# zubair-irshad/HunyuanWorld-Mirror

Hardware: AMD Instinct MI355X
Metric: views/sec (higher is better)
Workload: dtype bf16; 1 GPU; 8-view 518x518 bf16, no priors, camera+depth+pointmap+normal heads, 8 views/GPU, full 1.23B-param arch; views_per_gpu=8, global_views=8, parallelism=view-shard x1, collective=none (1 GPU)

## Files before the change

hunyuanworld-mirror_amd/csrc/elementwise.hip:

```cpp
#include "wm_common.h"
#include "wm_kernels.h"

namespace {

constexpr float RESNET_MEAN[3] = {0.485f, 0.456f, 0.406f};
constexpr float RESNET_STD[3] = {0.229f, 0.224f, 0.225f};

template <int NV>
__global__ __launch_bounds__(256) void layernorm_kernel(const WmLnArgs p) {
  const int lane = threadIdx.x & 63;
  const long long row = (long long)blockIdx.x * 4 + (threadIdx.x >> 6);
  const long long nrows = (long long)p.groups * p.rows_per_group;
  if (row >= nrows) return;
  const int g = (int)(row / p.rows_per_group), q = (int)(row - (long long)g * p.rows_per_group);
  const float* x = p.x + ((size_t)g * p.in_group + p.in_off + q) * p.ld_in;
  const size_t orow = (size_t)g * p.out_group + p.out_off + q;
  float4 v[NV];
  float s = 0.f;
#pragma unroll
  for (int i = 0; i < NV; ++i) {
    const int c = (i * 64 + lane) * 4;
    v[i] = c < p.D ? *(const float4*)(x + c) : make_float4(0, 0, 0, 0);
    s += v[i].x + v[i].y + v[i].z + v[i].w;
  }
// ... 153 lines not shown
#pragma unroll
        for (int i = 0; i < 4; ++i) {
          const float o = __shfl_xor(v[i], 4);
          v[i] = v[i] * c[i] + sign * o * s[i];
        }
      }
      if (which == 0) {
#pragma unroll
        for (int i = 0; i < 4; ++i) v[i] *= p.q_scale;
      }
    }
    uint2 u;
    u.x = (uint32_t)f2t<T>(v[0]) | ((uint32_t)f2t<T>(v[1]) << 16);
    u.y = (uint32_t)f2t<T>(v[2]) | ((uint32_t)f2t<T>(v[3]) << 16);
    u16* dst = (u16*)(which == 0 ? p.q : which == 1 ? p.k : p.v);
    if (head_ok) *(uint2*)(dst + obase) = u;
  }
}

template <int T>
__global__ __launch_bounds__(256) void im2col_kernel(const float* __restrict__ img, u16* __restrict__ out, int N, int C,
                                                     int H, int W, int ps, int Kpad, int normalize) {
  const int gh = H / ps, gw = W / ps, K = C * ps * ps;
  const size_t total = (size_t)N * gh * gw * Kpad;
  for (size_t i = (size_t)blockIdx.x * 256 + threadIdx.x; i < total; i += (size_t)gridDim.x * 256) {
    const int k = (int)(i % Kpad);
    const size_t r = i / Kpad;
    float v = 0.f;
    if (k < K) {
      const int c = k / (ps * ps), kk = k - c * ps * ps, ky = kk / ps, kx = kk - ky * ps;
      const int px = (int)(r % gw), py = (int)((r / gw) % gh), n = (int)(r / ((size_t)gw * gh));
      v = img[(((size_t)n * C + c) * H + py * ps + ky) * W + px * ps + kx];
      if (normalize) v = (v - RESNET_MEAN[c]) / RESNET_STD[c];
    }
    out[i] = f2t<T>(v);
  }
}

template <int T>
WM_NO_PACKED_FP32 __global__ __launch_bounds__(256) void im2col_rows_kernel(const float* __restrict__ img, u16* __restrict__ out, int N, int C,
                                                          int H, int W, int ps, int Kpad, int normalize) {
  extern __shared__ __attribute__((aligned(16))) u16 tile[];
  const int gh = H / ps, gw = W / ps, K = C * ps * ps;
  const int c = blockIdx.x % C, py = (blockIdx.x / C) % gh, n = blockIdx.x / (C * gh);
  const float mean = normalize ? RESNET_MEAN[c] : 0.f, sd = normalize ? RESNET_STD[c] : 1.f;
  const float* src = img + (((size_t)n * C + c) * H + (size_t)py * ps) * W;
  const int half = (ps * W) >> 1;
  for (int i = threadIdx.x; i < half; i += 256) {
    const float2 v = *(const float2*)(src + 2 * i);
    const float a = normalize ? (v.x - mean) / sd : v.x, b = normalize ? (v.y - mean) / sd : v.y;
    *(uint32_t*)(tile + 2 * i) = (uint32_t)f2t<T>(a) | ((uint32_t)f2t<T>(b) << 16);
  }
  __syncthreads();
  const int pp = ps * ps, hp = pp >> 1;
  u16* dst = out + ((size_t)n * gh * gw + (size_t)py * gw) * Kpad + (size_t)c * pp;
  for (int i = threadIdx.x; i < gw * hp; i += 256) {
    const int px = i / hp, kk = 2 * (i - px * hp), ky = kk / ps, kx = kk - ky * ps;
    *(uint32_t*)(dst + (size_t)px * Kpad + kk) = *(const uint32_t*)(tile + ky * W + px * ps + kx);
  }
  if (c == C - 1) {
    const int tail = (Kpad - K) >> 1;
    u16* z = out + ((size_t)n * gh * gw + (size_t)py * gw) * Kpad + K;
    for (int i = threadIdx.x; i < gw * tail; i += 256) {
      const int px = i / tail, j = i - px * tail;
      *(uint32_t*)(z + (size_t)px * Kpad + 2 * j) = 0u;
    }
  }
}

template <int T>
__global__ __launch_bounds__(256) void im2col7_kernel(const float* __restrict__ img, u16* __restrict__ out, int N, int H, int W,
                                                      int Kpad) {
  const size_t total = (size_t)N * H * W * Kpad;
  for (size_t i = (size_t)blockIdx.x * 256 + threadIdx.x; i < total; i += (size_t)gridDim.x * 256) {
    const int k = (int)(i % Kpad);
    const size_t r = i / Kpad;
    float v = 0.f;
    if (k < 147) {
      const int c = k / 49, kk = k - c * 49, ky = kk / 7, kx = kk - ky * 7;
      const int x = (int)(r % W), y = (int)((r / W) % H), n = (int)(r / ((size_t)W * H));
      const int iy = y + ky - 3, ix = x + kx - 3;
      if (iy >= 0 && iy < H && ix >= 0 && ix < W) v = img[(((size_t)n * 3 + c) * H + iy) * W + ix];
    }
    out[i] = f2t<T>(v);
  }
}

__global__ __launch_bounds__(256) void gs_splat_kernel(const float* __restrict__ gp, const float* __restrict__ img,
                                                       const float* __restrict__ depth, const float* __restrict__ cam,
                                                       float* __restrict__ means, float* __restrict__ quats,
                                                       float* __restrict__ scales, float* __restrict__ opac,
                                                       float* __restrict__ sh, float* __restrict__ wts, int N, int H, int W, int dbg) {
  const size_t npix = (size_t)N * H * W;
  for (size_t i = (size_t)blockIdx.x * 256 + threadIdx.x; i < npix; i += (size_t)gridDim.x * 256) {
    const int x = (int)(i % W), y = (int)((i / W) % H), n = (int)(i / ((size_t)W * H));
    const float* g = gp + i * 12;
    const float4 g0 = *(const float4*)g, g1 = *(const float4*)(g + 4), g2 = *(const float4*)(g + 8);
    const float qn = sqrtf(g0.x * g0.x + g0.y * g0.y + g0.z * g0.z + g0.w * g0.w) + 1e-8f;
    quats[i * 4 + 0] = g0.x / qn; quats[i * 4 + 1] = g0.y / qn; quats[i * 4 + 2] = g0.z / qn; quats[i * 4 + 3] = g0.w / qn;
    const float e0 = expf(g1.x), e1 = expf(g1.y), e2 = expf(g1.z);
    scales[i * 3 + 0] = e0 > 0.3f ? 0.3f : e0; scales[i * 3 + 1] = e1 > 0.3f ? 0.3f : e1; scales[i * 3 + 2] = e2 > 0.3f ? 0.3f : e2;
    opac[i] = 1.0f / (1.0f + expf(-g1.w));
    const float C0 = 0.28209479177387814f;
    const size_t hw = (size_t)H * W, p0 = (size_t)n * 3 * hw + (size_t)y * W + x;
    sh[i * 3 + 0] = (img[p0] - 0.5f) / C0 + g2.x;
    sh[i * 3 + 1] = (img[p0 + hw] - 0.5f) / C0 + g2.y;
    sh[i * 3 + 2] = (img[p0 + 2 * hw] - 0.5f) / C0 + g2.z;
    wts[i] = 1.0f / (1.0f + expf(-g2.w));
    const float* v = cam + n * 9;
    const float qi = v[3], qj = v[4], qk = v[5], qr = v[6];
    const float s2 = 2.0f / (qi * qi + qj * qj + qk * qk + qr * qr);
    const float R[9] = {1 - s2 * (qj * qj + qk * qk), s2 * (qi * qj - qk * qr), s2 * (qi * qk + qj * qr),
                        s2 * (qi * qj + qk * qr), 1 - s2 * (qi * qi + qk * qk), s2 * (qj * qk - qi * qr),
                        s2 * (qi * qk - qj * qr), s2 * (qj * qk + qi * qr), 1 - s2 * (qi * qi + qj * qj)};
    const float fy = H * 0.5f / tanf(v[7] * 0.5f), fx = W * 0.5f / tanf(v[8] * 0.5f);
    const float d = depth[i];
    const float xc = ((float)x - W * 0.5f) * d / fx, yc = ((float)y - H * 0.5f) * d / fy, zc = d;
    float tc[3];
    for (int a = 0; a < 3; ++a) tc[a] = -(R[0 * 3 + a] * v[0] + R[1 * 3 + a] * v[1] + R[2 * 3 + a] * v[2]);
    for (int a = 0; a < 3; ++a) means[i * 3 + a] = R[0 * 3 + a] * xc + R[1 * 3 + a] * yc + R[2 * 3 + a] * zc + tc[a];
#ifdef WM_DBG_SPLAT_BUILD
    if (dbg) {
      opac[i] = v[0]; wts[i] = v[1]; scales[i * 3 + 0] = v[2]; scales[i * 3 + 1] = v[7]; scales[i * 3 + 2] = v[8];
      quats[i * 4 + 0] = v[3]; quats[i * 4 + 1] = v[4]; quats[i * 4 + 2] = v[5]; quats[i * 4 + 3] = v[6];
      sh[i * 3 + 0] = tc[0]; sh[i * 3 + 1] = tc[1]; sh[i * 3 + 2] = tc[2];
    }
#else
    (void)dbg;
#endif
  }
}

__global__ __launch_bounds__(256) void dino_special_kernel(const float* cls, const float* reg, const float* pos, float* X,
                                                           int N, int T, int R, int D) {
  const int total = N * (1 + R) * D;
  for (int i = blockIdx.x * 256 + threadIdx.x; i < total; i += gridDim.x * 256) {
    const int d = i % D, t = (i / D) % (1 + R), n = i / (D * (1 + R));
    X[((size_t)n * T + t) * D + d] = t == 0 ? cls[d] + pos[d] : reg[(t - 1) * D + d];
  }
}

__global__ __launch_bounds__(256) void vgt_special_kernel(float* X, const float* cam, const float* reg, const float* pose,
                                                          const float* ray, int N, int P, int R, int D, int cond,
                                                          int first_view_global) {
  const int psi = 1 + R + (cond ? 2 : 0);
  const int total = N * psi * D;
  for (int i = blockIdx.x * 256 + threadIdx.x; i < total; i += gridDim.x * 256) {
    const int d = i % D, t = (i / D) % psi, n = i / (D * psi);
    const int slot = (first_view_global + n) == 0 ? 0 : 1;
    float v;
    if (t == 0) v = cam[slot * D + d];
    else if (t <= R) v = reg[(slot * R + (t - 1)) * D + d];
    else if (t == R + 1) v = pose ? pose[(size_t)n * D + d] : 0.f;
    else v = ray ? ray[(size_t)n * D + d] : 0.f;
    X[((size_t)n * P + t) * D + d] = v;
  }
}

__global__ __launch_bounds__(256) void copy2d_kernel(const float* __restrict__ src, float* __restrict__ dst, int rows,
                                                     int cols4, int ld_src, int ld_dst) {
  const size_t total = (size_t)rows * cols4;
  for (size_t i = (size_t)blockIdx.x * 256 + threadIdx.x; i < total; i += (size_t)gridDim.x * 256) {
    const size_t r = i / cols4;
    const int c = (int)(i - r * cols4) * 4;
    *(float4*)(dst + r * ld_dst + c) = *(const float4*)(src + r * ld_src + c);
  }
}

template <int OUT16>
__global__ __launch_bounds__(256) void bilinear_kernel(const float* __restrict__ in, void* __restrict__ outp, int N, int Hi,
                                                       int Wi, int Ho, int Wo, int C4, const float* __restrict__ addx,
                                                       const float* __restrict__ addy) {
  const float sy = Ho > 1 ? (float)(Hi - 1) / (float)(Ho - 1) : 0.f;
  const float sx = Wo > 1 ? (float)(Wi - 1) / (float)(Wo - 1) : 0.f;
  const size_t total = (size_t)N * Ho * Wo * C4;
  for (size_t i = (size_t)blockIdx.x * 256 + threadIdx.x; i < total; i += (size_t)gridDim.x * 256) {
    const int c = (int)(i % C4) * 4;
    size_t r = i / C4;
    const int x = (int)(r % Wo); r /= Wo;
    const int y = (int)(r % Ho);
    const int n = (int)(r / Ho);
    const float fy = sy * y, fx = sx * x;
    int y0 = (int)fy, x0 = (int)fx;
    y0 = y0 < Hi - 1 ? y0 : Hi - 1;
    x0 = x0 < Wi - 1 ? x0 : Wi - 1;
    const int y1 = y0 < Hi - 1 ? y0 + 1 : y0, x1 = x0 < Wi - 1 ? x0 + 1 : x0;
    const float wy = fy - y0, wx = fx - x0;
    const size_t C = (size_t)C4 * 4;
    const float* b = in + (size_t)n * Hi * Wi * C + c;
    const float4 v00 = *(const float4*)(b + ((size_t)y0 * Wi + x0) * C);
    const float4 v01 = *(const float4*)(b + ((size_t)y0 * Wi + x1) * C);
    const float4 v10 = *(const float4*)(b + ((size_t)y1 * Wi + x0) * C);
    const float4 v11 = *(const float4*)(b + ((size_t)y1 * Wi + x1) * C);
    const float w00 = (1.f - wy) * (1.f - wx), w01 = (1.f - wy) * wx, w10 = wy * (1.f - wx), w11 = wy * wx;
    float4 o;
    o.x = w00 * v00.x + w01 * v01.x + w10 * v10.x + w11 * v11.x;
    o.y = w00 * v00.y + w01 * v01.y + w10 * v10.y + w11 * v11.y;
    o.z = w00 * v00.z + w01 * v01.z + w10 * v10.z + w11 * v11.z;
    o.w = w00 * v00.w + w01 * v01.w + w10 * v10.w + w11 * v11.w;
    if (addx) {
      const int half = (int)(C >> 1);
      const float4 a = c < half ? *(const float4*)(addx + (size_t)x * half + c) : *(const float4*)(addy + (size_t)y * half + (c - half));
      o.x += a.x; o.y += a.y; o.z += a.z; o.w += a.w;
    }
    const size_t oi = (((size_t)n * Ho + y) * Wo + x) * C + c;
    if constexpr (OUT16 == 0) {
      *(float4*)((float*)outp + oi) = o;
    } else {
      uint2 u;
      if constexpr (OUT16 == 1) { u.x = (uint32_t)f2bf(o.x) | ((uint32_t)f2bf(o.y) << 16); u.y = (uint32_t)f2bf(o.z) | ((uint32_t)f2bf(o.w) << 16); }
      else { u.x = (uint32_t)f2h(o.x) | ((uint32_t)f2h(o.y) << 16); u.y = (uint32_t)f2h(o.z) | ((uint32_t)f2h(o.w) << 16); }
      *(uint2*)((u16*)outp + oi) = u;
    }
  }
}

constexpr int RT_P = 12;
template <int OUT16>
__global__ __launch_bounds__(256) void bilinear_tiled_kernel(const float* __restrict__ in, void* __restrict__ outp, int N, int Hi, int Wi,
                                                             int Ho, int Wo, int C, const float* __restrict__ addx,
                                                             const float* __restrict__ addy) {
  __shared__ __attribute__((aligned(16))) float patch[RT_P * RT_P * 64];
  const float sy = Ho > 1 ? (float)(Hi - 1) / (float)(Ho - 1) : 0.f;
  const float sx = Wo > 1 ? (float)(Wi - 1) / (float)(Wo - 1) : 0.f;
  const int tiles_x = (Wo + 15) / 16, tiles_y = (Ho + 15) / 16;
  int t = blockIdx.x;
  const int tx = t % tiles_x; t /= tiles_x;
  const int ty = t % tiles_y;
  const int n = t / tiles_y;
  const int y0 = ty * 16, x0 = tx * 16;
  const int y_last = min(y0 + 15, Ho - 1), x_last = min(x0 + 15, Wo - 1);
  auto lo = [](float s, int o, int lim) { int v = (int)(s * o); return v < lim - 1 ? v : lim - 1; };
  const int py0 = lo(sy, y0, Hi), px0 = lo(sx, x0, Wi);
  const int py1 = min(lo(sy, y_last, Hi) + 1, Hi - 1), px1 = min(lo(sx, x_last, Wi) + 1, Wi - 1);
  const int ph = py1 - py0 + 1, pw = px1 - px0 + 1;
  const int tid = threadIdx.x;
  const float* src = in + (size_t)n * Hi * Wi * C;
  for (int c0 = 0; c0 < C; c0 += 64) {
    __syncthreads();
    const int npieces = ph * pw * 16;
    for (int q = tid; q < npieces; q += 256) {
      const int pix = q >> 4, k = q & 15;
      const int yy = pix / pw, xx = pix - yy * pw;
      *(float4*)(patch + pix * 64 + k * 4) = *(const float4*)(src + ((size_t)(py0 + yy) * Wi + (px0 + xx)) * C + c0 + k * 4);
    }
    __syncthreads();
#pragma unroll 2
    for (int it = 0; it < 8; ++it) {
      const int item = it * 256 + tid, pix = item >> 3, g = item & 7;
      const int y = y0 + (pix >> 4), x = x0 + (pix & 15);
      if (y >= Ho || x >= Wo) continue;
      const float fy = sy * y, fx = sx * x;
      int ya = (int)fy, xa = (int)fx;
      ya = ya < Hi - 1 ? ya : Hi - 1;
      xa = xa < Wi - 1 ? xa : Wi - 1;
      const int yb = ya < Hi - 1 ? ya + 1 : ya, xb = xa < Wi - 1 ? xa + 1 : xa;
      const float wy = fy - ya, wx = fx - xa;
      const float w00 = (1.f - wy) * (1.f - wx), w01 = (1.f - wy) * wx, w10 = wy * (1.f - wx), w11 = wy * wx;
      const float* p00 = patch + ((ya - py0) * pw + (xa - px0)) * 64 + g * 8;
      const float* p01 = patch + ((ya - py0) * pw + (xb - px0)) * 64 + g * 8;
      const float* p10 = patch + ((yb - py0) * pw + (xa - px0)) * 64 + g * 8;
      const float* p11 = patch + ((yb - py0) * pw + (xb - px0)) * 64 + g * 8;
      float o[8];
#pragma unroll
      for (int h = 0; h < 2; ++h) {
        const float4 v00 = *(const float4*)(p00 + 4 * h), v01 = *(const float4*)(p01 + 4 * h);
        const float4 v10 = *(const float4*)(p10 + 4 * h), v11 = *(const float4*)(p11 + 4 * h);
        o[4 * h + 0] = w00 * v00.x + w01 * v01.x + w10 * v10.x + w11 * v11.x;
        o[4 * h + 1] = w00 * v00.y + w01 * v01.y + w10 * v10.y + w11 * v11.y;
        o[4 * h + 2] = w00 * v00.z + w01 * v01.z + w10 * v10.z + w11 * v11.z;
        o[4 * h + 3] = w00 * v00.w + w01 * v01.w + w10 * v10.w + w11 * v11.w;
      }
      const int c = c0 + g * 8;
      if (addx) {
        const int half = C >> 1;
        const float* a = c < half ? addx + (size_t)x * half + c : addy + (size_t)y * half + (c - half);
        const float4 a0 = *(const float4*)a, a1 = *(const float4*)(a + 4);
        o[0] += a0.x; o[1] += a0.y; o[2] += a0.z; o[3] += a0.w; o[4] += a1.x; o[5] += a1.y; o[6] += a1.z; o[7] += a1.w;
      }
      const size_t oi = (((size_t)n * Ho + y) * Wo + x) * C + c;
      if constexpr (OUT16 == 0) {
        *(float4*)((float*)outp + oi) = make_float4(o[0], o[1], o[2], o[3]);
        *(float4*)((float*)outp + oi + 4) = make_float4(o[4], o[5], o[6], o[7]);
      } else {
        uint4 u;
        if constexpr (OUT16 == 1) {
          u.x = (uint32_t)f2bf(o[0]) | ((uint32_t)f2bf(o[1]) << 16); u.y = (uint32_t)f2bf(o[2]) | ((uint32_t)f2bf(o[3]) << 16);
          u.z = (uint32_t)f2bf(o[4]) | ((uint32_t)f2bf(o[5]) << 16); u.w = (uint32_t)f2bf(o[6]) | ((uint32_t)f2bf(o[7]) << 16);
        } else {
          u.x = (uint32_t)f2h(o[0]) | ((uint32_t)f2h(o[1]) << 16); u.y = (uint32_t)f2h(o[2]) | ((uint32_t)f2h(o[3]) << 16);
          u.z = (uint32_t)f2h(o[4]) | ((uint32_t)f2h(o[5]) << 16); u.w = (uint32_t)f2h(o[6]) | ((uint32_t)f2h(o[7]) << 16);
        }
        *(uint4*)((u16*)outp + oi) = u;
      }
    }
  }
}
static bool bilinear_tiled_ok(int Hi, int Wi, int Ho, int Wo, int C) {
  if (C % 64 || Ho < 16 || Wo < 16) return false;
  const float sy = Ho > 1 ? (float)(Hi - 1) / (float)(Ho - 1) : 0.f, sx = Wo > 1 ? (float)(Wi - 1) / (float)(Wo - 1) : 0.f;
  return 15.f * sy + 3.f <= (float)RT_P && 15.f * sx + 3.f <= (float)RT_P;
}

__global__ __launch_bounds__(256) void add_kernel(const float* __restrict__ a, const float* __restrict__ b,
                                                  float* __restrict__ o, size_t n4) {
  for (size_t i = (size_t)blockIdx.x * 256 + threadIdx.x; i < n4; i += (size_t)gridDim.x * 256) {
    const float4 x = ((const float4*)a)[i], y = ((const float4*)b)[i];
    ((float4*)o)[i] = make_float4(x.x + y.x, x.y + y.y, x.z + y.z, x.w + y.w);
  }
}

__global__ __launch_bounds__(256) void dpt_tail_kernel(const float* __restrict__ y32, const float* __restrict__ w,
                                                       const float* __restrict__ b, float* __restrict__ attr,
                                                       float* __restrict__ conf, size_t npix, int C, int act) {
  __shared__ float sw[4 * 32 + 4];
  if (threadIdx.x < C * 32) sw[threadIdx.x] = w[threadIdx.x];
  if (threadIdx.x < C) sw[128 + threadIdx.x] = b[threadIdx.x];
  __syncthreads();
  for (size_t i = (size_t)blockIdx.x * 256 + threadIdx.x; i < npix; i += (size_t)gridDim.x * 256) {
    float o[4] = {sw[128], sw[129], sw[130], sw[131]};
    const float4* src = (const float4*)(y32 + i * 32);
#pragma unroll
    for (int k = 0; k < 8; ++k) {
      float4 v = src[k];
      v.x = relu_keep_nan(v.x); v.y = relu_keep_nan(v.y); v.z = relu_keep_nan(v.z); v.w = relu_keep_nan(v.w);
#pragma unroll
      for (int c = 0; c < 4; ++c)
        if (c < C) o[c] += v.x * sw[c * 32 + 4 * k] + v.y * sw[c * 32 + 4 * k + 1] + v.z * sw[c * 32 + 4 * k + 2] + v.w * sw[c * 32 + 4 * k + 3];
    }
    const int A = C - 1;
    if (act == WM_ACT_NORM) {
      float nn = 0.f;
      for (int c = 0; c < A; ++c) nn += o[c] * o[c];
      nn = sqrtf(nn);
      for (int c = 0; c < A; ++c) attr[i * A + c] = o[c] / nn;
    } else if (act == WM_ACT_EXP) {
      for (int c = 0; c < A; ++c) attr[i * A + c] = expf(o[c]);
    } else {
      for (int c = 0; c < A; ++c) attr[i * A + c] = inv_log(o[c]);
    }
    conf[i] = 1.0f + expf(o[A]);
  }
}

inline int grid_for(size_t n, int per_block = 256) {
  size_t g = (n + per_block - 1) / per_block;
  return (int)(g < 1 ? 1 : (g > 2048 ? 2048 : g));
}

}

hipError_t wm_launch_layernorm(const WmLnArgs& a, hipStream_t s) {
  const long long rows = (long long)a.groups * a.rows_per_group;
  if (rows <= 0) return hipSuccess;
  if (a.D % 4 || a.D > 2048 || a.ld_in % 4 || a.ld_out % 4) return hipErrorInvalidValue;
  dim3 grid((unsigned)((rows + 3) / 4)), block(256);
  const int nv = (a.D + 255) / 256;
  if (a.D == nv * 256 && (nv == 4 || nv == 8) && !a.w && !a.b && !a.out_f32) {
    if (nv == 4) {
      if (a.dtype == WM_T_BF16) hipLaunchKernelGGL((layernorm_fast_noaffine_kernel<4, WM_T_BF16>), grid, block, 0, s, a);
      else hipLaunchKernelGGL((layernorm_fast_noaffine_kernel<4, WM_T_F16>), grid, block, 0, s, a);
    } else {
      if (a.dtype == WM_T_BF16) hipLaunchKernelGGL((layernorm_fast_noaffine_kernel<8, WM_T_BF16>), grid, block, 0, s, a);
      else hipLaunchKernelGGL((layernorm_fast_noaffine_kernel<8, WM_T_F16>), grid, block, 0, s, a);
    }
    return hipGetLastError();
  }
  if (a.D == nv * 256 && (nv == 4 || nv == 8) && a.w && a.b && !a.out_f32) {
    const int rpw = nv == 4 && wm_tune(WM_TUNE_LN_RPW, 1) == 2 ? 2 : 1;
    const dim3 g2((unsigned)((rows + 4 * rpw - 1) / (4 * rpw)));
    if (nv == 4 && rpw == 2) {
      if (a.dtype == WM_T_BF16) hipLaunchKernelGGL((layernorm_fast_kernel<4, WM_T_BF16, 2>), g2, block, 0, s, a);
      else hipLaunchKernelGGL((layernorm_fast_kernel<4, WM_T_F16, 2>), g2, block, 0, s, a);
    } else if (nv == 4) {
      if (a.dtype == WM_T_BF16) hipLaunchKernelGGL((layernorm_fast_kernel<4, WM_T_BF16, 1>), grid, block, 0, s, a);
      else hipLaunchKernelGGL((layernorm_fast_kernel<4, WM_T_F16, 1>), grid, block, 0, s, a);
    } else {
      if (a.dtype == WM_T_BF16) hipLaunchKernelGGL((layernorm_fast_kernel<8, WM_T_BF16, 1>), grid, block, 0, s, a);
      else hipLaunchKernelGGL((layernorm_fast_kernel<8, WM_T_F16, 1>), grid, block, 0, s, a);
    }
    return hipGetLastError();
  }
  if (nv <= 1) hipLaunchKernelGGL(layernorm_kernel<1>, grid, block, 0, s, a);
  else if (nv <= 2) hipLaunchKernelGGL(layernorm_kernel<2>, grid, block, 0, s, a);
  else if (nv <= 4) hipLaunchKernelGGL(layernorm_kernel<4>, grid, block, 0, s, a);
  else hipLaunchKernelGGL(layernorm_kernel<8>, grid, block, 0, s, a);
  return hipGetLastError();
}

hipError_t wm_launch_qkv_post(const WmQkvArgs& a, hipStream_t s) {
  if (a.M <= 0) return hipSuccess;
  const long long waves = (long long)a.M * ((a.H + 3) / 4);
  dim3 grid((unsigned)((waves + 3) / 4)), block(256);
  if (a.dtype == WM_T_BF16) hipLaunchKernelGGL(qkv_post_kernel<WM_T_BF16>, grid, block, 0, s, a);
  else hipLaunchKernelGGL(qkv_post_kernel<WM_T_F16>, grid, block, 0, s, a);
  return hipGetLastError();
}

hipError_t wm_launch_im2col(const float* img, void* out, int N, int C, int H, int W, int ps, int Kpad, int normalize,
                            int dtype, hipStream_t s) {
  const size_t total = (size_t)N * (H / ps) * (W / ps) * Kpad;
  if (!total) return hipSuccess;
  const size_t lds = (size_t)ps * W * sizeof(u16);
  if (ps % 2 == 0 && W % 2 == 0 && (C * ps * ps) % 2 == 0 && Kpad % 2 == 0 && lds <= 64 * 1024) {
    const dim3 grid((unsigned)(N * (H / ps) * C));
    if (dtype == WM_T_BF16) hipLaunchKernelGGL(im2col_rows_kernel<WM_T_BF16>, grid, dim3(256), lds, s, img, (u16*)out, N, C, H, W, ps, Kpad, normalize);
    else hipLaunchKernelGGL(im2col_rows_kernel<WM_T_F16>, grid, dim3(256), lds, s, img, (u16*)out, N, C, H, W, ps, Kpad, normalize);
    return hipGetLastError();
  }
  if (dtype == WM_T_BF16)
    hipLaunchKernelGGL(im2col_kernel<WM_T_BF16>, dim3(grid_for(total)), dim3(256), 0, s, img, (u16*)out, N, C, H, W, ps, Kpad, normalize);
  else
    hipLaunchKernelGGL(im2col_kernel<WM_T_F16>, dim3(grid_for(total)), dim3(256), 0, s, img, (u16*)out, N, C, H, W, ps, Kpad, normalize);
  return hipGetLastError();
}

hipError_t wm_launch_im2col7(const float* img, void* out, int N, int H, int W, int Kpad, int dtype, hipStream_t s) {
  const size_t total = (size_t)N * H * W * Kpad;
  if (!total) return hipSuccess;
  if (dtype == WM_T_BF16) hipLaunchKernelGGL(im2col7_kernel<WM_T_BF16>, dim3(grid_for(total)), dim3(256), 0, s, img, (u16*)out, N, H, W, Kpad);
  else hipLaunchKernelGGL(im2col7_kernel<WM_T_F16>, dim3(grid_for(total)), dim3(256), 0, s, img, (u16*)out, N, H, W, Kpad);
  return hipGetLastError();
}

hipError_t wm_launch_gs_splat(const float* gp, const float* img, const float* depth, const float* cam, float* means, float* quats,
                              float* scales, float* opac, float* sh, float* wts, int N, int H, int W, hipStream_t s) {
  if (!N) return hipSuccess;
#ifdef WM_DBG_SPLAT_BUILD
  const int dbg = wm_tune(WM_TUNE_DBG_SPLAT, 0) ? 1 : 0;
#else
  const int dbg = 0;
#endif
  hipLaunchKernelGGL(gs_splat_kernel, dim3(grid_for((size_t)N * H * W)), dim3(256), 0, s, gp, img, depth, cam, means, quats, scales,
                     opac, sh, wts, N, H, W, dbg);
  return hipGetLastError();
}

hipError_t wm_launch_dino_tokens(const float* , const float* cls, const float* reg, const float* pos, float* X,
                                 int N, int hw, int R, int D, hipStream_t s) {
  hipLaunchKernelGGL(dino_special_kernel, dim3(grid_for((size_t)N * (1 + R) * D)), dim3(256), 0, s, cls, reg, pos, X, N,
                     1 + R + hw, R, D);
  return hipGetLastError();
}

hipError_t wm_launch_vgt_special(float* X, const float* cam_tok, const float* reg_tok, const float* pose_tok,
                                 const float* ray_tok, int N, int P, int R, int D, int cond, int first_view_global,
                                 hipStream_t s) {
  hipLaunchKernelGGL(vgt_special_kernel, dim3(grid_for((size_t)N * (3 + R) * D)), dim3(256), 0, s, X, cam_tok, reg_tok,
                     pose_tok, ray_tok, N, P, R, D, cond, first_view_global);
  return hipGetLastError();
}

hipError_t wm_launch_copy2d(const float* src, float* dst, int rows, int cols, int ld_src, int ld_dst, hipStream_t s) {
  if (cols % 4 || ld_src % 4 || ld_dst % 4) return hipErrorInvalidValue;
  if (!rows) return hipSuccess;
  hipLaunchKernelGGL(copy2d_kernel, dim3(grid_for((size_t)rows * cols / 4)), dim3(256), 0, s, src, dst, rows, cols / 4, ld_src, ld_dst);
  return hipGetLastError();
}

hipError_t wm_launch_bilinear(const float* in, float* out, int N, int Hi, int Wi, int Ho, int Wo, int C, const float* addx,
                              const float* addy, hipStream_t s) {
  if (C % 8) return hipErrorInvalidValue;
  const size_t total = (size_t)N * Ho * Wo * (C / 4);
  if (!total) return hipSuccess;
  if (bilinear_tiled_ok(Hi, Wi, Ho, Wo, C)) {
    hipLaunchKernelGGL(bilinear_tiled_kernel<0>, dim3((unsigned)(N * ((Ho + 15) / 16) * ((Wo + 15) / 16))), dim3(256), 0, s, in, (void*)out, N, Hi, Wi, Ho, Wo, C, addx, addy);
    return hipGetLastError();
  }
  hipLaunchKernelGGL(bilinear_kernel<0>, dim3(grid_for(total)), dim3(256), 0, s, in, (void*)out, N, Hi, Wi, Ho, Wo, C / 4, addx, addy);
  return hipGetLastError();
}

hipError_t wm_launch_bilinear16(const float* in, void* out16, int N, int Hi, int Wi, int Ho, int Wo, int C, const float* addx,
                                const float* addy, int dtype, hipStream_t s) {
  if (C % 4) return hipErrorInvalidValue;
  const size_t total = (size_t)N * Ho * Wo * (C / 4);
  if (!total) return hipSuccess;
  if (bilinear_tiled_ok(Hi, Wi, Ho, Wo, C)) {
    const dim3 grid((unsigned)(N * ((Ho + 15) / 16) * ((Wo + 15) / 16)));
    if (dtype == WM_T_BF16) hipLaunchKernelGGL(bilinear_tiled_kernel<1>, grid, dim3(256), 0, s, in, out16, N, Hi, Wi, Ho, Wo, C, addx, addy);
    else hipLaunchKernelGGL(bilinear_tiled_kernel<2>, grid, dim3(256), 0, s, in, out16, N, Hi, Wi, Ho, Wo, C, addx, addy);
    return hipGetLastError();
  }
  if (dtype == WM_T_BF16) hipLaunchKernelGGL(bilinear_kernel<1>, dim3(grid_for(total)), dim3(256), 0, s, in, out16, N, Hi, Wi, Ho, Wo, C / 4, addx, addy);
  else hipLaunchKernelGGL(bilinear_kernel<2>, dim3(grid_for(total)), dim3(256), 0, s, in, out16, N, Hi, Wi, Ho, Wo, C / 4, addx, addy);
  return hipGetLastError();
}

hipError_t wm_launch_add(const float* a, const float* b, float* out, size_t n, hipStream_t s) {
  if (n % 4) return hipErrorInvalidValue;
  if (!n) return hipSuccess;
  hipLaunchKernelGGL(add_kernel, dim3(grid_for(n / 4)), dim3(256), 0, s, a, b, out, n / 4);
  return hipGetLastError();
}

template <int VEC>
__global__ __launch_bounds__(256) void depth_to_world_kernel(const float* __restrict__ depth, const float* __restrict__ ext,
                                                             const float* __restrict__ intr, float* __restrict__ world,
                                                             float* __restrict__ cam, unsigned char* __restrict__ mask, int B,
                                                             int H, int W, float eps) {
  const size_t hw = (size_t)H * W, total = (size_t)B * hw / VEC;
  for (size_t i = (size_t)blockIdx.x * 256 + threadIdx.x; i < total; i += (size_t)gridDim.x * 256) {
    float zz[VEC], cw[3 * VEC], cc[3 * VEC];
    if constexpr (VEC == 4) {
      const float4 d4 = *(const float4*)(depth + 4 * i);
      zz[0] = d4.x; zz[1] = d4.y; zz[2] = d4.z; zz[3] = d4.w;
    } else {
      zz[0] = depth[i];
    }
    unsigned int mbits = 0;
#pragma unroll
    for (int e = 0; e < VEC; ++e) {
      const size_t px = VEC * i + e;
      const int b = (int)(px / hw);
      const size_t r = px - (size_t)b * hw;
      const int v = (int)(r / W), u = (int)(r - (size_t)v * W);
      const float* K = intr + b * 9;
      const float* E = ext + b * 16;
      const float z = zz[e];
      const float x = __fdiv_rn(__fmul_rn((float)u - K[2], z), K[0]);
      const float y = __fdiv_rn(__fmul_rn((float)v - K[5], z), K[4]);
      cc[3 * e] = x; cc[3 * e + 1] = y; cc[3 * e + 2] = z;
#pragma unroll
      for (int j = 0; j < 3; ++j) cw[3 * e + j] = E[4 * j] * x + E[4 * j + 1] * y + E[4 * j + 2] * z + E[4 * j + 3];
      mbits |= (z > eps ? 1u : 0u) << (8 * e);
    }
    if constexpr (VEC == 4) {
      if (cam) {
#pragma unroll
        for (int q = 0; q < 3; ++q) *(float4*)(cam + 12 * i + 4 * q) = make_float4(cc[4 * q], cc[4 * q + 1], cc[4 * q + 2], cc[4 * q + 3]);
      }
      if (world) {
#pragma unroll
        for (int q = 0; q < 3; ++q) *(float4*)(world + 12 * i + 4 * q) = make_float4(cw[4 * q], cw[4 * q + 1], cw[4 * q + 2], cw[4 * q + 3]);
      }
      if (mask) *(unsigned int*)(mask + 4 * i) = mbits;
    } else {
      if (cam) { cam[3 * i] = cc[0]; cam[3 * i + 1] = cc[1]; cam[3 * i + 2] = cc[2]; }
      if (world) { world[3 * i] = cw[0]; world[3 * i + 1] = cw[1]; world[3 * i + 2] = cw[2]; }
      if (mask) mask[i] = (unsigned char)mbits;
    }
  }
}

hipError_t wm_launch_depth_to_world(const float* depth, const float* ext, const float* intr, float* world, float* cam,
                                    unsigned char* mask, int B, int H, int W, float eps, hipStream_t s) {
  const size_t total = (size_t)B * H * W;
  if (!total) return hipSuccess;
  const bool al = (((size_t)depth | (size_t)world | (size_t)cam) & 15) == 0 && ((size_t)mask & 3) == 0;
  if (total % 4 == 0 && al)
    hipLaunchKernelGGL(depth_to_world_kernel<4>, dim3(grid_for(total / 4)), dim3(256), 0, s, depth, ext, intr, world, cam, mask, B, H, W, eps);
  else
    hipLaunchKernelGGL(depth_to_world_kernel<1>, dim3(grid_for(total)), dim3(256), 0, s, depth, ext, intr, world, cam, mask, B, H, W, eps);
  return hipGetLastError();
}

hipError_t wm_launch_dpt_tail(const float* y32, const float* w, const float* b, float* attr, float* conf, size_t npix,
                              int C, int act, hipStream_t s) {
  if (C < 2 || C > 4) return hipErrorInvalidValue;
  if (!npix) return hipSuccess;
  hipLaunchKernelGGL(dpt_tail_kernel, dim3(grid_for(npix)), dim3(256), 0, s, y32, w, b, attr, conf, npix, C, act);
  return hipGetLastError();
}
```

hunyuanworld-mirror_amd/csrc/wm_kernels.h:

```cpp
#pragma once
#include <hip/hip_runtime.h>
#include <stdint.h>
#include <stddef.h>


enum {
  WM_EPI_F32 = 0,
  WM_EPI_T16 = 1,
  WM_EPI_GELU_T16 = 2,
  WM_EPI_RESID = 3,
  WM_EPI_ROWMAP_ADD = 4,
  WM_EPI_CONVT = 5,
  WM_EPI_QKV = 6,
  WM_EPI_CONV = 7,
};

struct WmQkvArgs {
  const float* qkv; void* q; void* k; void* v;
  const float* qn_w; const float* qn_b; const float* kn_w; const float* kn_b;
  const float* rope_cos; const float* rope_sin;
  int M, H, head_stride;
  int tokens_per_view, patch_start, grid_w;
  float inv_tpv, inv_gw;
  float q_scale; int dtype;
// ... 16 lines not shown
  int cv_h, cv_w, cv_cin;
  const void* cv_zero;
  const float* cv_resid; const float* cv_resid2;
  int cv_resid_relu;
  int tc_k;
  unsigned tc_list[16];
  void* ln_out; int ln_ld;
  const float* ln_w; const float* ln_b; float ln_eps;
  float* ln_stats;
  int* ln_sync;
  int* ln_fallback;
};
hipError_t wm_launch_gemm(const WmGemmArgs& a, hipStream_t s);
bool wm_gemm_fuses_ln(const WmGemmArgs& a);
hipError_t wm_launch_gemm_ln_fallback(const WmGemmArgs& a, hipStream_t s);

#define WM_ATTN_MAX_SPLITS_C 8
struct WmAttnArgs {
  const void* Q; const void* K; const void* V;
  void* O;
  int H;
  int q_rows;
  int seq_len;
  int q_head_stride;
  int kv_head_stride;
  int kv_chunks;
  long long kv_chunk_stride;
  int kv_rows_per_chunk;
  int dtype;
  int kv_splits, max_splits;
  int full_units;
  float* part_o; float* part_ml;
  int* unit_flags;
  const int* only_if;
  int* unit_hint;
  int* unit_stat;
  int force_partial, part_slot0;
};
hipError_t wm_launch_attention_combine(const WmAttnArgs& a, int slots, hipStream_t s);
hipError_t wm_launch_attention(const WmAttnArgs& a, hipStream_t s);
int wm_attention_variant(const WmAttnArgs& a);
void wm_attention_geometry(const WmAttnArgs& a, int* unit_rows, int* blocks_per_cu);
hipError_t wm_launch_attention_v3(const WmAttnArgs& a, int grid, int* flags, hipStream_t s);
hipError_t wm_launch_attention_v4(const WmAttnArgs& a, int grid, int* flags, hipStream_t s);
inline size_t wm_attention_max_blocks(int q_rows, int seq_len, int H) {
  const size_t nseq = (size_t)(q_rows / (seq_len > 0 ? seq_len : 1));
  return ((size_t)(seq_len + 127) / 128 + 1) * nseq * (size_t)H * WM_ATTN_MAX_SPLITS_C;
}
constexpr int WM_ATTN_MAX_SPLITS = 8;
constexpr int WM_ATTN_HINT_TTL = 15;

struct WmLnArgs {
  const float* x; void* y; const float* w; const float* b;
  int D, ld_in, ld_out; float eps;
  int groups, rows_per_group, in_group, in_off, out_group, out_off;
  int out_f32, dtype;
};
hipError_t wm_launch_layernorm(const WmLnArgs& a, hipStream_t s);

hipError_t wm_launch_qkv_post(const WmQkvArgs& a, hipStream_t s);

hipError_t wm_launch_im2col(const float* img, void* out, int N, int C, int H, int W, int ps, int Kpad,
                            int normalize, int dtype, hipStream_t s);
hipError_t wm_launch_im2col7(const float* img, void* out, int N, int H, int W, int Kpad, int dtype, hipStream_t s);
hipError_t wm_launch_gs_splat(const float* gp, const float* img, const float* depth, const float* cam, float* means, float* quats,
                              float* scales, float* opac, float* sh, float* wts, int N, int H, int W, hipStream_t s);
hipError_t wm_launch_dino_tokens(const float* patch, const float* cls, const float* reg, const float* pos,
                                 float* X, int N, int hw, int R, int D, hipStream_t s);
hipError_t wm_launch_vgt_special(float* X, const float* cam_tok, const float* reg_tok, const float* pose_tok,
                                 const float* ray_tok, int N, int P, int R, int D, int cond, int first_view_global,
                                 hipStream_t s);
hipError_t wm_launch_copy2d(const float* src, float* dst, int rows, int cols, int ld_src, int ld_dst, hipStream_t s);
hipError_t wm_launch_bilinear(const float* in, float* out, int N, int Hi, int Wi, int Ho, int Wo, int C,
                              const float* addx, const float* addy, hipStream_t s);
hipError_t wm_launch_add(const float* a, const float* b, float* out, size_t n, hipStream_t s);
hipError_t wm_launch_depth_to_world(const float* depth, const float* ext, const float* intr, float* world, float* cam,
                                    unsigned char* mask, int B, int H, int W, float eps, hipStream_t s);
hipError_t wm_launch_resample_h(const unsigned char* in, unsigned char* out, int H, int Wi, int Wo, const int* bounds, const int* kk,
                                int ksize, hipStream_t s);
hipError_t wm_launch_resample_v_tensor(const unsigned char* tmp, float* out, int Hi, int W, int Ho, int Hf, int Wf, int ry0, int rx0,
                                       const int* bounds, const int* kk, int ksize, hipStream_t s);
size_t wm_confidence_mask_workspace(size_t n);
hipError_t wm_launch_confidence_mask(const float* conf, size_t n, unsigned int K, unsigned char* mask, void* workspace, hipStream_t s);
hipError_t wm_launch_depth_edge(const float* depth, const unsigned char* mask, int S, int H, int W, int k, int has_atol, float atol,
                                int has_rtol, float rtol, unsigned char* out, hipStream_t s);
hipError_t wm_launch_normals_edge(const float* normals, const unsigned char* mask, int S, int H, int W, int k, double tol_deg,
                                  unsigned char* out, hipStream_t s);
size_t wm_point_filter_mask_workspace(int S, int H, int W);
hipError_t wm_launch_point_filter_mask(const float* conf, const float* depth, const float* normals, int S, int H, int W, int apply_conf,
                                       double percentile, int apply_edge, double normal_tol_deg, float depth_rtol,
                                       float* thresholds_out, unsigned char* mask_out, unsigned char* out_de, unsigned char* out_ne,
                                       void* ws, hipStream_t s);
hipError_t wm_launch_dpt_tail(const float* y32, const float* w, const float* b, float* attr, float* conf,
                              size_t npix, int C, int act, hipStream_t s);
enum { WM_ACT_INV_LOG = 0, WM_ACT_EXP = 1, WM_ACT_NORM = 2 };

struct WmConvArgs {
  const float* x;
  const void* w;
  const float* bias;
  const float* resid;
  const float* resid2;
  float* y;
  int N, Hi, Wi, Cin, Ho, Wo, Cout, ksize, stride, pad;
  int relu_in, resid_relu, relu_out, dtype;
  int up_hs, up_ws;
  const float* up_addx; const float* up_addy;
  int out16;
  int in16;
  int dbg;
};
bool wm_conv3x3_applicable(const WmConvArgs& a);
bool wm_conv3x3_out16_ok(const WmConvArgs& a);
struct WmConvN32Args {
  const uint16_t* x; const uint16_t* w; const float* bias; float* y; const uint16_t* zero;
  int N, H, W, Cin, relu_out, dtype;
  const float* tail_w; const float* tail_b; float* tail_attr; float* tail_conf; int tail_C, tail_act;
};
hipError_t wm_launch_conv3x3_n32_in16(const WmConvN32Args& a, hipStream_t s);
hipError_t wm_launch_bilinear16(const float* in, void* out16, int N, int Hi, int Wi, int Ho, int Wo, int C, const float* addx,
                                const float* addy, int dtype, hipStream_t s);
hipError_t wm_launch_conv(const WmConvArgs& a, hipStream_t s);
hipError_t wm_launch_f32_to_16_2d(const float* src, int ld_src, void* dst16, int ld_dst, int rows, int cols, int dtype, hipStream_t s);
hipError_t wm_launch_tconv_border(float* out, const float* bmiss, int N, int H, int W, int F, hipStream_t s);
hipError_t wm_launch_repack_tap_major(const void* w16, void* wt16, int Co, int C, hipStream_t s);
hipError_t wm_launch_upconv_gather(const void* y16, const float* bias, float* out, int N, int Hi, int Wi, int Ho, int Wo, int Co, hipStream_t s);

hipError_t wm_launch_linear_f32(const float* X, const float* W, const float* b, float* Y, int M, int N, int K,
                                int ldx, int ldy, int pre_act, int post_act, const float* gamma, int accumulate,
                                hipStream_t s);
hipError_t wm_launch_small_attention(const float* qkv, float* out, int S, int heads, int hd, hipStream_t s);
hipError_t wm_launch_adaln(const float* tok, const float* mod, float* h, int S, int D, float eps, hipStream_t s);
hipError_t wm_launch_cam_update(float* pred, const float* delta, float* out, int S, int first, hipStream_t s);
hipError_t wm_launch_cam_matrices(const float* params, float* poses, float* intrs, int S, int H, int W, hipStream_t s);

#ifndef WM_COLORS_PER_CAMERA
#define WM_COLORS_PER_CAMERA 2
#endif
struct WmRasterArgs {
  const float* means; const float* quats; const float* scales; const float* opacities;
  const float* colors; int is_sh;
  int N;
  int sh_degree, n_coeffs; const float* campos;
  const float* viewmats; const float* Ks; int C;
  int width, height;
  float* out_rgb; float* out_depth; float* out_alpha;
  int* radii_out;
  void* workspace; size_t workspace_bytes; size_t max_isects;
  int antialiased;
  int depth_mode;
  float eps2d, near_plane, far_plane, radius_clip;
  const float* backgrounds;
};
inline void wm_raster_default_options(WmRasterArgs& a) {
  a.antialiased = 0; a.depth_mode = 0; a.eps2d = 0.3f; a.near_plane = 0.01f; a.far_plane = 1e10f; a.radius_clip = 0.f; a.backgrounds = nullptr;
}
inline bool wm_raster_options_valid(const WmRasterArgs& a) {
  return (a.antialiased == 0 || a.antialiased == 1) && (a.depth_mode == 0 || a.depth_mode == 1) && a.eps2d >= 0.f && a.near_plane < a.far_plane &&
         a.radius_clip >= 0.f;
}
size_t wm_raster_workspace_bytes(int N, int C, int width, int height, size_t max_isects);
hipError_t wm_launch_rasterize(const WmRasterArgs& a, hipStream_t s, unsigned long long* n_isects_out);
struct WmRasterBwdArgs {
  WmRasterArgs fwd;
  size_t n_isects;
  const float* out_depth;
  const float* v_rgb; const float* v_depth; const float* v_alpha;
  float* v_means; float* v_quats; float* v_scales; float* v_opacities; float* v_colors;
  void* grad_workspace; size_t grad_workspace_bytes;
  float* v_means2d; float* v_means2d_abs; int absgrad;
  float* v_viewmats;
  float* v_campos;
  float* v_backgrounds; const float* out_alpha;
};
size_t wm_raster_bwd_workspace_bytes(int N, int C, int width, int height, size_t n_isects, int absgrad = 0, int cam = 0, int sh = 0, int campos = 0,
                                     int bg = 0);
hipError_t wm_launch_rasterize_bwd(const WmRasterBwdArgs& b, hipStream_t s);
hipError_t wm_launch_rasterize_means2d(const void* workspace, size_t workspace_bytes, int N, int C, int width, int height, size_t max_isects,
                                       const int* radii, float* means2d, hipStream_t s);

struct WmDensifyPlanArgs {
  const float* grad2d; const float* count; const float* radii_state;
  const float* scales; const float* opacities;
  int N;
  float grow_grad2d, grow_scale3d, grow_scale2d, prune_opa, prune_scale3d, prune_scale2d;
  int use_scale2d, prune_big, revised_opacity;
  int* src; int* kind; int* rank;
  int* counts;
  void* workspace; size_t workspace_bytes;
};
enum { WM_DENSIFY_KEEP = 0, WM_DENSIFY_DUP = 1, WM_DENSIFY_SPLIT0 = 2, WM_DENSIFY_SPLIT1 = 3 };
enum { WM_GATHER_COPY = 0, WM_GATHER_ZERO_NEW = 1, WM_GATHER_MEANS = 2, WM_GATHER_SCALES = 3, WM_GATHER_OPACITIES_REVISED = 4 };
hipError_t wm_launch_densify_accumulate(const float* v_means2d, const int* radii, int N, int C, int width, int height, float* grad2d,
                                        float* count, float* radii_state, hipStream_t s);
size_t wm_densify_plan_ws_bytes(size_t N);
hipError_t wm_launch_densify_plan(const WmDensifyPlanArgs& a, hipStream_t s);
hipError_t wm_launch_densify_gather(const float* in, float* out, int N, int R, int mode, const int* src, const int* kind, const int* rank,
                                    int n_out, const float* quats, const float* scales, const float* noise, hipStream_t s);

hipError_t wm_launch_mcmc_inject_noise(float* means, const float* quats, const float* scales, const float* opacities, const float* noise,
                                       float scaler, int N, hipStream_t s);
size_t wm_mcmc_partition_ws_bytes(size_t N);
hipError_t wm_launch_mcmc_partition(const float* opacities, const unsigned char* mask, int N, float min_opacity, int* dead_idx, int* alive_idx,
                                    int* counts_host, void* workspace, size_t workspace_bytes, hipStream_t s);
hipError_t wm_launch_mcmc_relocation(const float* opacities, const float* scales, const int* sampled, int n_sampled, int N, float min_opacity,
                                     float* new_opacities, float* new_scales, int* hist, hipStream_t s);
hipError_t wm_launch_mcmc_scatter(float* t, int rows, int R, const int* sampled, const int* dest, const float* values, int n_sampled,
                                  hipStream_t s);
hipError_t wm_launch_mcmc_zero_rows(float* t, int rows, int R, const int* idx, int n, hipStream_t s);

struct WmPhotoLossArgs {
  const float* img1; const float* img2;
  const int64_t* strides1; const int64_t* strides2;
  int B, C, H, W, padding_valid;
  void* workspace; size_t workspace_bytes;
};
size_t wm_photoloss_workspace_bytes(int B, int C, int H, int W);
size_t wm_photoloss_forward_only_bytes(int B, int H, int W);
hipError_t wm_launch_photoloss_fwd(const WmPhotoLossArgs& a, int want_backward, float* out_ssim, float* out_l1, hipStream_t s);
hipError_t wm_launch_photoloss_bwd(const WmPhotoLossArgs& a, const float* g_ssim, const float* g_l1, float* grad_img1, hipStream_t s);

constexpr int WM_BILAGRID_MAX_CELLS = 4096;
struct WmBilagridArgs {
  const float* grids; const int* grid_idx; const float* xy; const float* rgb;
  int G, L, Hg, Wg, B, n;
};
size_t wm_bilagrid_bwd_workspace_bytes(int G, int L, int Hg, int Wg, int B, int n);
hipError_t wm_launch_bilagrid_slice(const WmBilagridArgs& a, float* out, hipStream_t s);
hipError_t wm_launch_bilagrid_slice_bwd(const WmBilagridArgs& a, const float* v_out, float* v_grids, float* v_rgb, void* ws, size_t ws_bytes,
                                        hipStream_t s);
size_t wm_bilagrid_tv_ws_bytes(int B, int C, int L, int H, int W);
hipError_t wm_launch_bilagrid_tv(const float* x, int B, int C, int L, int H, int W, float* out, void* ws, size_t ws_bytes, hipStream_t s);
hipError_t wm_launch_bilagrid_tv_bwd(const float* x, int B, int C, int L, int H, int W, const float* g, float* v_x, hipStream_t s);

struct WmDepthLossArgs {
  const float* depth; const int64_t* strides;
  const float* points; const float* depth_gt; const unsigned char* valid;
  int C, H, W, M;
  void* workspace; size_t workspace_bytes;
};
size_t wm_depthloss_workspace_bytes(int C, int H, int W, int M, int want_backward);
hipError_t wm_launch_depthloss_fwd(const WmDepthLossArgs& a, int want_backward, float* out, hipStream_t s);
hipError_t wm_launch_depthloss_bwd(const WmDepthLossArgs& a, const float* gout, float* v_depth, const int64_t* v_strides, hipStream_t s);
hipError_t wm_launch_depth_project(const float* points_world, const float* camtoworlds, const float* Ks, const unsigned char* visible, int C, int P,
                                   int W, int H, float* points, float* depths, unsigned char* valid, hipStream_t s);

constexpr int WM_APPEARANCE_TILE = 128;
constexpr int WM_APPEARANCE_MAX_BLOCKS = 512;
struct WmAppearanceArgs {
  const float* features;
  const float* embeds; const int* embed_ids;
  const float* dirs;
  const float* W1; const float* b1; const float* W2; const float* b2; const float* W3; const float* b3;
  int N, C, n_embeds, n_bases, degree;
};
struct WmAppearanceGrads {
  const float* v_out;
  float* v_features; float* v_dirs;
  float* v_embeds;
  float* v_W1; float* v_b1; float* v_W2; float* v_b2; float* v_W3; float* v_b3;
};
size_t wm_appearance_bwd_workspace_bytes(int N, int C);
hipError_t wm_launch_appearance_fwd(const WmAppearanceArgs& a, float* out, hipStream_t s);
hipError_t wm_launch_appearance_bwd(const WmAppearanceArgs& a, const WmAppearanceGrads& v, void* ws, size_t ws_bytes, hipStream_t s);

size_t wm_prune_workspace_bytes(size_t N);
hipError_t wm_launch_prune_gs(const float* means, const float* quats, const float* scales, const float* opac, const float* sh,
                              const float* weights, int N, float voxel, float* o_means, float* o_quats, float* o_scales, float* o_opac,
                              float* o_sh, int* K_out, void* workspace, size_t ws_bytes, hipStream_t s);

#define WM_TUNE_KEYS(X) \
  X(GEMM_CFG, "gemm_cfg") \
  X(GEMM_PP, "gemm_pp") \
  X(GEMM_MFMA16, "gemm_mfma16") \
  X(ATTN_QB, "attn_qb") \
  X(OP_LDPAD, "op_ldpad") \
  X(ATTN_SPLITS, "attn_splits") \
  X(CONV_FUSE_UP, "conv_fuse_up") \
  X(CONV_NARROW, "conv_narrow") \
  X(CONV_BN, "conv_bn") \
  X(CONV_RS, "conv_rs") \
  X(LIN_MFMA, "lin_mfma") \
  X(CONV_TPX, "conv_tpx") \
  X(ATTN_TAIL, "attn_tail") \
  X(GEMM_GROUP, "gemm_group") \
  X(COMM_OVERLAP, "comm_overlap") \
  X(HEADS_CONC, "heads_concurrent") \
  X(RCU_MID16, "rcu_mid16") \
  X(GEMM_SCHED, "gemm_sched") \
  X(FORCE_GATHER, "force_gather") \
  X(ATTN_OP_POLICY, "attn_op_policy") \
  X(COMM_P2P, "comm_p2p") \
  X(LN_RPW, "ln_rpw") \
  X(LN_FUSE, "ln_fuse") \
  X(HEADS_MAIN, "heads_main") \
  X(CONV_GEMM, "conv_gemm") \
  X(RESID_PREFETCH, "resid_prefetch") \
  X(UP1_GATHER, "up1_gather") \
  X(TCONV, "tconv") \
  X(UP1_COMP, "up1_comp") \
  X(CONV_BM, "conv_bm") \
  X(RASTER_PPL, "raster_ppl") \
  X(TAP_SHARED, "tap_shared") \
  X(ATTN_DEBUG_SKIP, "attn_debug_skip") \
  X(CONV_DBG, "conv_dbg") \
  X(DBG_SPLAT, "dbg_splat")
#define WM_TUNE_ENUM(name_, key_) WM_TUNE_##name_,
enum { WM_TUNE_KEYS(WM_TUNE_ENUM) WM_TUNE_COUNT };
#undef WM_TUNE_ENUM
extern int wm_tuning[WM_TUNE_COUNT];
inline int wm_tune(int key, int dflt) { return wm_tuning[key] < 0 ? dflt : wm_tuning[key]; }
```

Baseline: 159.8 views/s.

## Add persistent software-pipelined tiled bilinear resize kernel with nontemporal stores

Adds a v2 tiled bilinear upsample kernel, enabled by default. It splits work into 64-channel chunks per 16x16 output tile and makes blocks persistent, each handling several items. The next item's source patch and add-table are prefetched into registers while the current one computes from shared memory. Large outputs use nontemporal stores to avoid polluting cache. This adds register pressure and a more complex indexing path, and only affects the resize portion of the DPT heads.

```diff
diff --git a/hunyuanworld-mirror_amd/csrc/elementwise.hip b/hunyuanworld-mirror_amd/csrc/elementwise.hip
--- a/hunyuanworld-mirror_amd/csrc/elementwise.hip
+++ b/hunyuanworld-mirror_amd/csrc/elementwise.hip
@@ -479,6 +479,139 @@
   return 15.f * sy + 3.f <= (float)RT_P && 15.f * sx + 3.f <= (float)RT_P;
 }
 
+typedef float rt_f4 __attribute__((ext_vector_type(4)));
+typedef uint32_t rt_u4 __attribute__((ext_vector_type(4)));
+constexpr int RT_NLOAD = RT_P * RT_P * 16 / 256;
+struct RtItem { int n, y0, x0, py0, px0, ph, pw, c0; };
+template <int OUT16, bool NT>
+__global__ __launch_bounds__(256, 4) void bilinear_tiled_v2_kernel(const float* __restrict__ in, void* __restrict__ outp, int N, int Hi, int Wi,
+                                                                int Ho, int Wo, int C, const float* __restrict__ addx,
+                                                                const float* __restrict__ addy, int per, int nitems) {
+  __shared__ __attribute__((aligned(16))) float patch[RT_P * RT_P * 64];
+  __shared__ __attribute__((aligned(16))) float tab[16 * 64];
+  const float sy = Ho > 1 ? (float)(Hi - 1) / (float)(Ho - 1) : 0.f;
+  const float sx = Wo > 1 ? (float)(Wi - 1) / (float)(Wo - 1) : 0.f;
+  const int tiles_x = (Wo + 15) / 16, tiles_y = (Ho + 15) / 16, nchunk = C / 64, half = C >> 1;
+  const int tid = threadIdx.x;
+  auto item_of = [&](int w) {
+    RtItem g;
+    int t = w / nchunk;
+    g.c0 = (w - t * nchunk) * 64;
+    const int tx = t % tiles_x; t /= tiles_x;
+    const int ty = t % tiles_y;
+    g.n = t / tiles_y;
+    g.y0 = ty * 16; g.x0 = tx * 16;
+    const int y_last = min(g.y0 + 15, Ho - 1), x_last = min(g.x0 + 15, Wo - 1);
+    auto lo = [](float s, int o, int lim) { int v = (int)(s * o); return v < lim - 1 ? v : lim - 1; };
+    g.py0 = lo(sy, g.y0, Hi); g.px0 = lo(sx, g.x0, Wi);
+    const int py1 = min(lo(sy, y_last, Hi) + 1, Hi - 1), px1 = min(lo(sx, x_last, Wi) + 1, Wi - 1);
+    g.ph = py1 - g.py0 + 1; g.pw = px1 - g.px0 + 1;
+    return g;
+  };
+  rt_f4 r[RT_NLOAD], rtab;
+  auto fetch = [&](const RtItem& g) {
+    const int npieces = g.ph * g.pw * 16;
+    const uint32_t inv = 65536u / (uint32_t)g.pw + 1u;
+    const float* src = in + (size_t)g.n * Hi * Wi * C + g.c0;
+#pragma unroll
+    for (int j = 0; j < RT_NLOAD; ++j) {
+      const int q = min(j * 256 + tid, npieces - 1);
+      const int pix = q >> 4, k = q & 15;
+      const int yy = (int)(((uint32_t)pix * inv) >> 16), xx = pix - yy * g.pw;
+      r[j] = *(const rt_f4*)(src + ((size_t)(g.py0 + yy) * Wi + (g.px0 + xx)) * C + k * 4);
+    }
+    const int pos = tid >> 4, c = g.c0 + (tid & 15) * 4;
+    const bool isx = c < half;
+    const int p = min((isx ? g.x0 : g.y0) + pos, (isx ? Wo : Ho) - 1);
+    const float* tsrc = addx ? (isx ? addx + (size_t)p * half + c : addy + (size_t)p * half + (c - half)) : src;
+    rtab = *(const rt_f4*)tsrc;
+  };
+  int w = blockIdx.x * per;
+  const int w_end = min(w + per, nitems);
+  if (w >= w_end) return;
+  RtItem g = item_of(w);
+  fetch(g);
+  for (; w < w_end; ++w) {
+    __syncthreads();
+    {
+      const int npieces = g.ph * g.pw * 16;
+#pragma unroll
+      for (int j = 0; j < RT_NLOAD; ++j) {
+        const int q = j * 256 + tid;
+        if (q < npieces) *(rt_f4*)(patch + q * 4) = r[j];
+      }
+      *(rt_f4*)(tab + tid * 4) = rtab;
+    }
+    __syncthreads();
+    const RtItem gn = w + 1 < w_end ? item_of(w + 1) : g;
+    if (w + 1 < w_end) fetch(gn);
+    const int y0 = g.y0, x0 = g.x0, py0 = g.py0, px0 = g.px0, pw = g.pw, c0 = g.c0, n = g.n;
+#pragma unroll 2
+    for (int it = 0; it < 8; ++it) {
+      const int item = it * 256 + tid, pix = item >> 3, gq = item & 7;
+      const int y = y0 + (pix >> 4), x = x0 + (pix & 15);
+      if (y >= Ho || x >= Wo) continue;
+      const float fy = sy * y, fx = sx * x;
+      int ya = (int)fy, xa = (int)fx;
+      ya = ya < Hi - 1 ? ya : Hi - 1;
+      xa = xa < Wi - 1 ? xa : Wi - 1;
+      const int yb = ya < Hi - 1 ? ya + 1 : ya, xb = xa < Wi - 1 ? xa + 1 : xa;
+      const float wy = fy - ya, wx = fx - xa;
+      const float w00 = (1.f - wy) * (1.f - wx), w01 = (1.f - wy) * wx, w10 = wy * (1.f - wx), w11 = wy * wx;
+      const float* p00 = patch + ((ya - py0) * pw + (xa - px0)) * 64 + gq * 8;
+      const float* p01 = patch + ((ya - py0) * pw + (xb - px0)) * 64 + gq * 8;
+      const float* p10 = patch + ((yb - py0) * pw + (xa - px0)) * 64 + gq * 8;
+      const float* p11 = patch + ((yb - py0) * pw + (xb - px0)) * 64 + gq * 8;
+      float o[8];
+#pragma unroll
+      for (int h = 0; h < 2; ++h) {
+        const float4 v00 = *(const float4*)(p00 + 4 * h), v01 = *(const float4*)(p01 + 4 * h);
+        const float4 v10 = *(const float4*)(p10 + 4 * h), v11 = *(const float4*)(p11 + 4 * h);
+        o[4 * h + 0] = w00 * v00.x + w01 * v01.x + w10 * v10.x + w11 * v11.x;
+        o[4 * h + 1] = w00 * v00.y + w01 * v01.y + w10 * v10.y + w11 * v11.y;
+        o[4 * h + 2] = w00 * v00.z + w01 * v01.z + w10 * v10.z + w11 * v11.z;
+        o[4 * h + 3] = w00 * v00.w + w01 * v01.w + w10 * v10.w + w11 * v11.w;
+      }
+      const int c = c0 + gq * 8;
+      if (addx) {
+        const float* a = tab + (c < half ? (pix & 15) : (pix >> 4)) * 64 + gq * 8;
+        const float4 a0 = *(const float4*)a, a1 = *(const float4*)(a + 4);
+        o[0] += a0.x; o[1] += a0.y; o[2] += a0.z; o[3] += a0.w; o[4] += a1.x; o[5] += a1.y; o[6] += a1.z; o[7] += a1.w;
+      }
+      const size_t oi = (((size_t)n * Ho + y) * Wo + x) * C + c;
+      if constexpr (OUT16 == 0) {
+        rt_f4 s0, s1;
+        s0.x = o[0]; s0.y = o[1]; s0.z = o[2]; s0.w = o[3]; s1.x = o[4]; s1.y = o[5]; s1.z = o[6]; s1.w = o[7];
+        if constexpr (NT) {
+          __builtin_nontemporal_store(s0, (rt_f4*)((float*)outp + oi));
+          __builtin_nontemporal_store(s1, (rt_f4*)((float*)outp + oi + 4));
+        } else {
+          *(rt_f4*)((float*)outp + oi) = s0;
+          *(rt_f4*)((float*)outp + oi + 4) = s1;
+        }
+      } else {
+        rt_u4 u;
+        if constexpr (OUT16 == 1) {
+          u.x = (uint32_t)f2bf(o[0]) | ((uint32_t)f2bf(o[1]) << 16); u.y = (uint32_t)f2bf(o[2]) | ((uint32_t)f2bf(o[3]) << 16);
+          u.z = (uint32_t)f2bf(o[4]) | ((uint32_t)f2bf(o[5]) << 16); u.w = (uint32_t)f2bf(o[6]) | ((uint32_t)f2bf(o[7]) << 16);
+        } else {
+          u.x = (uint32_t)f2h(o[0]) | ((uint32_t)f2h(o[1]) << 16); u.y = (uint32_t)f2h(o[2]) | ((uint32_t)f2h(o[3]) << 16);
+          u.z = (uint32_t)f2h(o[4]) | ((uint32_t)f2h(o[5]) << 16); u.w = (uint32_t)f2h(o[6]) | ((uint32_t)f2h(o[7]) << 16);
+        }
+        if constexpr (NT) __builtin_nontemporal_store(u, (rt_u4*)((u16*)outp + oi));
+        else *(rt_u4*)((u16*)outp + oi) = u;
+      }
+    }
+    g = gn;
+  }
+}
+constexpr size_t RT_NT_BYTES = (size_t)256 << 20;
+static void bilinear_v2_grid(int N, int Ho, int Wo, int C, int* per, int* nitems, unsigned* grid) {
+  *nitems = N * ((Ho + 15) / 16) * ((Wo + 15) / 16) * (C / 64);
+  *per = (*nitems + 1023) / 1024;
+  *grid = (unsigned)((*nitems + *per - 1) / *per);
+}
+
 __global__ __launch_bounds__(256) void add_kernel(const float* __restrict__ a, const float* __restrict__ b,
                                                   float* __restrict__ o, size_t n4) {
   for (size_t i = (size_t)blockIdx.x * 256 + threadIdx.x; i < n4; i += (size_t)gridDim.x * 256) {
@@ -641,6 +774,13 @@
   const size_t total = (size_t)N * Ho * Wo * (C / 4);
   if (!total) return hipSuccess;
   if (bilinear_tiled_ok(Hi, Wi, Ho, Wo, C)) {
+    if (wm_tune(WM_TUNE_RESIZE_V2, 1)) {
+      int per, nitems; unsigned grid;
+      bilinear_v2_grid(N, Ho, Wo, C, &per, &nitems, &grid);
+      if (total * 16 > RT_NT_BYTES) hipLaunchKernelGGL((bilinear_tiled_v2_kernel<0, true>), dim3(grid), dim3(256), 0, s, in, (void*)out, N, Hi, Wi, Ho, Wo, C, addx, addy, per, nitems);
+      else hipLaunchKernelGGL((bilinear_tiled_v2_kernel<0, false>), dim3(grid), dim3(256), 0, s, in, (void*)out, N, Hi, Wi, Ho, Wo, C, addx, addy, per, nitems);
+      return hipGetLastError();
+    }
     hipLaunchKernelGGL(bilinear_tiled_kernel<0>, dim3((unsigned)(N * ((Ho + 15) / 16) * ((Wo + 15) / 16))), dim3(256), 0, s, in, (void*)out, N, Hi, Wi, Ho, Wo, C, addx, addy);
     return hipGetLastError();
   }
@@ -654,6 +794,18 @@
   const size_t total = (size_t)N * Ho * Wo * (C / 4);
   if (!total) return hipSuccess;
   if (bilinear_tiled_ok(Hi, Wi, Ho, Wo, C)) {
+    if (wm_tune(WM_TUNE_RESIZE_V2, 1)) {
+      int per, nitems; unsigned g2;
+      bilinear_v2_grid(N, Ho, Wo, C, &per, &nitems, &g2);
+      if (total * 8 > RT_NT_BYTES) {
+        if (dtype == WM_T_BF16) hipLaunchKernelGGL((bilinear_tiled_v2_kernel<1, true>), dim3(g2), dim3(256), 0, s, in, out16, N, Hi, Wi, Ho, Wo, C, addx, addy, per, nitems);
+        else hipLaunchKernelGGL((bilinear_tiled_v2_kernel<2, true>), dim3(g2), dim3(256), 0, s, in, out16, N, Hi, Wi, Ho, Wo, C, addx, addy, per, nitems);
+      } else {
+        if (dtype == WM_T_BF16) hipLaunchKernelGGL((bilinear_tiled_v2_kernel<1, false>), dim3(g2), dim3(256), 0, s, in, out16, N, Hi, Wi, Ho, Wo, C, addx, addy, per, nitems);
+        else hipLaunchKernelGGL((bilinear_tiled_v2_kernel<2, false>), dim3(g2), dim3(256), 0, s, in, out16, N, Hi, Wi, Ho, Wo, C, addx, addy, per, nitems);
+      }
+      return hipGetLastError();
+    }
     const dim3 grid((unsigned)(N * ((Ho + 15) / 16) * ((Wo + 15) / 16)));
     if (dtype == WM_T_BF16) hipLaunchKernelGGL(bilinear_tiled_kernel<1>, grid, dim3(256), 0, s, in, out16, N, Hi, Wi, Ho, Wo, C, addx, addy);
     else hipLaunchKernelGGL(bilinear_tiled_kernel<2>, grid, dim3(256), 0, s, in, out16, N, Hi, Wi, Ho, Wo, C, addx, addy);
diff --git a/hunyuanworld-mirror_amd/csrc/wm_kernels.h b/hunyuanworld-mirror_amd/csrc/wm_kernels.h
--- a/hunyuanworld-mirror_amd/csrc/wm_kernels.h
+++ b/hunyuanworld-mirror_amd/csrc/wm_kernels.h
@@ -342,6 +342,7 @@
   X(CONV_BM, "conv_bm") \
   X(RASTER_PPL, "raster_ppl") \
   X(TAP_SHARED, "tap_shared") \
+  X(RESIZE_V2, "resize_v2") \
   X(ATTN_DEBUG_SKIP, "attn_debug_skip") \
   X(CONV_DBG, "conv_dbg") \
   X(DBG_SPLAT, "dbg_splat")
```

Result: no change. 160.2 views/s, median of 3 (+0.2%).
